# douban/gobeansdb

Hardware: AMD Instinct MI355X
Metric: GiB/s device-resident QuickLZ decompress (+compress), batched 4-64 KiB values (higher is better)
Workload: dtype u8; 1 GPU; c2: decompress 1048576 x 16384 B text-like blocks per GPU (ratio 0.502), device-resident; blocks_per_gpu=1048576, block_size=16384, unique_blocks=1048576, fused_crc=False, parallelism=shard1

## Files before the change

### gobeansdb_amd/csrc/qlzx_decode_batch.h

```cpp
#pragma once
#include "qlzx_device.h"

#ifndef QLZX_FAST_MAX_DSIZE
#define QLZX_FAST_MAX_DSIZE 65536
#endif

namespace qlzx {

struct BlkInfo {
    uint32_t ngroups;
    uint32_t nitems;
    uint32_t kind;
    uint32_t dsize;
};
struct GroupRec {
    uint32_t ip, m, a, b;
};

constexpr int32_t kPending = -1;
constexpr uint32_t kBlkSkip = 0, kBlkStored = 1, kBlkCompressed = 2;
constexpr uint32_t kParseWG = 64;
#ifndef QLZX_CHUNK_BLOCKS
#define QLZX_CHUNK_BLOCKS 262144
#endif
#ifndef QLZX_CHUNK_BLOCKS_MIXED
#define QLZX_CHUNK_BLOCKS_MIXED 131072
#endif
__host__ __device__ inline uint32_t chunk_blocks(uint32_t max_dsize) {
    return max_dsize <= 16384 ? (uint32_t)QLZX_CHUNK_BLOCKS : (uint32_t)QLZX_CHUNK_BLOCKS_MIXED;
}
constexpr uint32_t kRoundBytes = 32;
constexpr uint32_t kPieces = kRoundBytes / 16;
#ifndef QLZX_K1_SLOTS
#define QLZX_K1_SLOTS 4
#endif
constexpr uint32_t kRingSlots = QLZX_K1_SLOTS;
template <uint32_t S>
constexpr uint32_t kRingWaveS = S * kRoundBytes * 64;
__host__ __device__ inline uint32_t groups_max(uint32_t max_dsize) { return max_dsize / 31u + 2u; }

struct BatchLayout {
    uint32_t md, gmax;
    uint32_t chunk, nchunks;
    size_t o_rec, o_list, o_aux;
    size_t one;
    uint32_t regions;
};
inline BatchLayout batch_layout(uint32_t n, uint32_t max_dsize) {
    auto a256 = [](size_t x) { return (x + 255) & ~(size_t)255; };
    BatchLayout L;
    L.md = max_dsize > QLZX_FAST_MAX_DSIZE ? QLZX_FAST_MAX_DSIZE : max_dsize;
    L.gmax = groups_max(L.md);
    const uint32_t cb = chunk_blocks(max_dsize);
    L.chunk = n < cb ? (n ? n : 1) : cb;
    L.nchunks = n <= cb ? 1u : 1u + (n - 1) / cb;
    L.o_rec = a256((size_t)L.chunk * sizeof(BlkInfo));
    L.o_list = L.o_rec + a256((size_t)L.chunk * L.gmax * sizeof(GroupRec));
    L.o_aux = L.o_list + a256((size_t)n * sizeof(uint32_t));
    L.one = L.o_aux + 1024 + 256;
    L.regions = L.nchunks == 1 ? 1u : max_dsize > 16384 && L.nchunks >= 3 ? 3u : 2u;
    return L;
}

__device__ __forceinline__ int classify_block(const uint8_t *src, uint32_t len, uint32_t cap, uint32_t max_dsize,
                                              uint32_t &kind, uint32_t &csize, uint32_t &dsize, uint32_t &hdr) {
    kind = kBlkSkip;
    if (len < 3) return QLZX_E_HEADER;
    hdr = (src[0] & 2u) ? 9u : 3u;
    if (len < hdr) return QLZX_E_HEADER;
    const Header h = parse_header(src);
    csize = h.csize;
    dsize = h.dsize;
    if (h.csize != len) return QLZX_E_SIZE_COMPRESSED;
    if (h.level != 3) return QLZX_E_LEVEL;
    if (h.dsize > cap) return QLZX_E_DST_CAP;
    if (h.dsize > max_dsize) return QLZX_E_MAX_DSIZE;
    if (h.dsize > QLZX_FAST_MAX_DSIZE) return kPending;
    if (!h.compressed) {
        if (csize < hdr + dsize) return QLZX_E_CORRUPT;
        kind = kBlkStored;
    } else {
        kind = kBlkCompressed;
    }
    return QLZX_OK;
}

template <uint32_t S>
__device__ __forceinline__ uint32_t ring_off(uint32_t q, uint32_t lane) {
    return (((q >> 4) & (kPieces * S - 1)) << 10) | (lane << 4) | (q & 15u);
}
template <uint32_t S>
__device__ __forceinline__ uint32_t ring_rd32(const uint8_t *ring, uint32_t q, uint32_t lane) {
    const uint32_t qa = q & ~3u;
    const uint32_t lo = *(const uint32_t *)(ring + ring_off<S>(qa, lane));
    const uint32_t hi = *(const uint32_t *)(ring + ring_off<S>(qa + 4, lane));
    return __builtin_amdgcn_alignbyte(hi, lo, q & 3u);
}

struct ItemCursor {
    uint32_t g, k;
    __device__ __forceinline__ void next() {
        k += 2;
        const bool wrap = k >= 31;
        k = wrap ? k - 31 : k;
        g += wrap ? 3 : 2;
    }
};

__device__ __forceinline__ void decode_tok_bf(uint32_t t, uint32_t &off, uint32_t &len, uint32_t &tl) {
    const uint32_t ty = (t & 3u) + ((t & 127u) == 3u ? 1u : 0u);
    const uint32_t f4 = ty * 4, f6 = ty * 6;
    const uint32_t osh = __builtin_amdgcn_ubfe(0xF7622u, f4, 4);
    const uint32_t ow = __builtin_amdgcn_ubfe((6u) | (14u << 6) | (10u << 12) | (17u << 18) | (17u << 24), f6, 6);
    const uint32_t lsh = __builtin_amdgcn_ubfe(0x72200u, f4, 4);
    const uint32_t lw = __builtin_amdgcn_ubfe(0x85400u, f4, 4);
    const uint32_t la = __builtin_amdgcn_ubfe(0x32333u, f4, 4);
    tl = __builtin_amdgcn_ubfe(0x43221u, f4, 4);
    off = __builtin_amdgcn_ubfe(t, osh, ow);
    len = __builtin_amdgcn_ubfe(t, lsh, lw) + la;
}

__device__ __forceinline__ uint32_t wave_incl_scan(uint32_t v) {
    v += (uint32_t)__builtin_amdgcn_update_dpp(0, (int)v, 0x111, 0xf, 0xf, true);
    v += (uint32_t)__builtin_amdgcn_update_dpp(0, (int)v, 0x112, 0xf, 0xf, true);
    v += (uint32_t)__builtin_amdgcn_update_dpp(0, (int)v, 0x114, 0xf, 0xf, true);
    v += (uint32_t)__builtin_amdgcn_update_dpp(0, (int)v, 0x118, 0xf, 0xf, true);
    v += (uint32_t)__builtin_amdgcn_update_dpp(0, (int)v, 0x142, 0xa, 0xf, false);
    v += (uint32_t)__builtin_amdgcn_update_dpp(0, (int)v, 0x143, 0xc, 0xf, false);
    return v;
}

constexpr int kIcmpNe = 33, kIcmpUlt = 36;
__device__ __forceinline__ uint64_t cmp_lt(uint32_t a, uint32_t b) { return __builtin_amdgcn_uicmp(a, b, kIcmpUlt); }
__device__ __forceinline__ uint64_t cmp_ne(uint32_t a, uint32_t b) { return __builtin_amdgcn_uicmp(a, b, kIcmpNe); }
__device__ __forceinline__ bool in_mask(uint64_t m) { return __builtin_amdgcn_inverse_ballot_w64(m); }

__device__ __forceinline__ uint32_t ff1_or(uint64_t m, uint32_t dflt) {
    return m ? (uint32_t)__builtin_ctzll(m) : dflt;
}

__device__ __forceinline__ uint32_t wave_incl_max(uint32_t v) {
    v = max(v, (uint32_t)__builtin_amdgcn_update_dpp(0, (int)v, 0x111, 0xf, 0xf, false));
    v = max(v, (uint32_t)__builtin_amdgcn_update_dpp(0, (int)v, 0x112, 0xf, 0xf, false));
    v = max(v, (uint32_t)__builtin_amdgcn_update_dpp(0, (int)v, 0x114, 0xf, 0xf, false));
    v = max(v, (uint32_t)__builtin_amdgcn_update_dpp(0, (int)v, 0x118, 0xf, 0xf, false));
    v = max(v, (uint32_t)__builtin_amdgcn_update_dpp(0, (int)v, 0x142, 0xa, 0xf, false));
    v = max(v, (uint32_t)__builtin_amdgcn_update_dpp(0, (int)v, 0x143, 0xc, 0xf, false));
    return v;
}
__device__ __forceinline__ uint32_t wave_shr1(uint32_t v) {
    return (uint32_t)__builtin_amdgcn_update_dpp(0, (int)v, 0x138, 0xf, 0xf, true);
}

}
```

### gobeansdb_amd/csrc/qlzx_decode_batch.hip

```cpp
#include "qlzx_decode_batch.h"
#include "qlzx_decode_k2.h"
#include "qlzx_host.h"

namespace qlzx {

constexpr uint32_t kOrderClasses = 128, kOrderWG = 64, kOrderEPT = 16, kOrderPerWG = kOrderWG * kOrderEPT;
constexpr uint32_t kOrderAux = 2 * kOrderClasses;
__device__ __forceinline__ uint32_t order_class(uint32_t len) {
    const uint32_t c = len >> 9;
    return c < kOrderClasses - 1 ? c : kOrderClasses - 1;
}
__global__ void __launch_bounds__(kOrderWG) k_order_count(const uint32_t *src_len, uint32_t n, uint32_t *aux) {
    __shared__ uint32_t h[kOrderClasses];
    const uint32_t tid = threadIdx.x, i0 = blockIdx.x * kOrderPerWG + tid;
    for (uint32_t k = tid; k < kOrderClasses; k += kOrderWG) h[k] = 0;
    __syncthreads();
    uint32_t len[kOrderEPT];
#pragma unroll
    for (uint32_t e = 0; e < kOrderEPT; e++) {
        const uint32_t i = i0 + e * kOrderWG;
        len[e] = i < n ? src_len[i] : 0u;
    }
#pragma unroll
    for (uint32_t e = 0; e < kOrderEPT; e++)
        if (i0 + e * kOrderWG < n) atomicAdd(&h[order_class(len[e])], 1u);
    __syncthreads();
    for (uint32_t k = tid; k < kOrderClasses; k += kOrderWG)
        if (h[k]) atomicAdd(&aux[k], h[k]);
}
__global__ void __launch_bounds__(kOrderWG) k_order_scatter(const uint32_t *src_len, uint32_t n, uint32_t *aux,
                                                           uint32_t *list) {
    __shared__ uint32_t start[kOrderClasses], lc[kOrderClasses];
    const uint32_t tid = threadIdx.x, i0 = blockIdx.x * kOrderPerWG + tid;
    for (uint32_t k = tid; k < kOrderClasses; k += kOrderWG) start[k] = aux[k], lc[k] = 0;
    __syncthreads();
    if (tid == 0) {
        uint32_t acc = 0;
        for (uint32_t k = 0; k < kOrderClasses; k++) {
            const uint32_t v = start[k];
            start[k] = acc;
            acc += v;
        }
    }
    uint32_t c[kOrderEPT], r[kOrderEPT];
#pragma unroll
    for (uint32_t e = 0; e < kOrderEPT; e++) {
        const uint32_t i = i0 + e * kOrderWG;
        c[e] = i < n ? order_class(src_len[i]) : 0u;
    }
#pragma unroll
    for (uint32_t e = 0; e < kOrderEPT; e++)
        r[e] = (i0 + e * kOrderWG < n) ? atomicAdd(&lc[c[e]], 1u) : 0u;
    __syncthreads();
    for (uint32_t k = tid; k < kOrderClasses; k += kOrderWG)
        if (lc[k]) start[k] += atomicAdd(&aux[kOrderClasses + k], lc[k]);
    __syncthreads();
#pragma unroll
    for (uint32_t e = 0; e < kOrderEPT; e++)
        if (i0 + e * kOrderWG < n) list[start[c[e]] + r[e]] = i0 + e * kOrderWG;
}

#ifndef QLZX_K1_KMAX_UNI
#define QLZX_K1_KMAX_UNI 12
#endif
#ifndef QLZX_K1_KMAX_MIX
#define QLZX_K1_KMAX_MIX 10
#endif
int launch_k1_parse6(uint32_t grid, hipStream_t s, const qlzx_blocks &b, const uint32_t *dst_cap, uint32_t *dsize,
                     int32_t *status, uint32_t first, uint32_t cnt, BlkInfo *info, GroupRec *recs, uint32_t gmax,
                     const uint32_t *order, uint32_t max_dsize, uint32_t kmax);
int launch_k2_nocrc(uint32_t grid, hipStream_t s, const qlzx_blocks &b, uint32_t *dsize, int32_t *status,
                    uint32_t first, uint32_t cnt, const BlkInfo *info, const GroupRec *recs, uint32_t gmax,
                    const uint32_t *order);
inline std::atomic<int> g_batch_fault{0};
inline int batch_fault(int kernel) {
    int k = kernel;
    return g_batch_fault.load(std::memory_order_relaxed) == kernel && g_batch_fault.compare_exchange_strong(k, 0)
               ? (int)hipErrorLaunchFailure
               : 0;
}

struct Side {
    hipStream_t st = nullptr, st2 = nullptr;
    hipEvent_t k1[2] = {}, k2[2] = {}, order = nullptr, last = nullptr;
    ~Side() {
        if (!st || g_hip_down.load()) return;
        for (int j = 0; j < 2; j++) {
            if (k1[j]) (void)hipEventDestroy(k1[j]);
            if (k2[j]) (void)hipEventDestroy(k2[j]);
        }
        if (order) (void)hipEventDestroy(order);
        if (last) (void)hipEventDestroy(last);
        if (st2) (void)hipStreamDestroy(st2);
        (void)hipStreamDestroy(st);
    }
};
inline int batch_side(hipStream_t s, Side *&out) {
    thread_local Side sides[kMaxDevices];
    int dev = 0, cur = 0;
    if (s) {
        hipDevice_t hd;
        if (hipStreamGetDevice(s, &hd) != hipSuccess) return (int)hipErrorInvalidResourceHandle;
        dev = (int)hd;
    } else if (hipGetDevice(&dev) != hipSuccess) {
        return (int)hipErrorNoDevice;
    }
    if (dev < 0 || dev >= (int)kMaxDevices) return (int)hipErrorInvalidDevice;
    Side &sd = sides[dev];
    if (!sd.st) {
        note_hip_up();
        (void)hipGetDevice(&cur);
        if (cur != dev) (void)hipSetDevice(dev);
        hipError_t e = hipStreamCreateWithFlags(&sd.st, hipStreamNonBlocking);
        if (e == hipSuccess) e = hipStreamCreateWithFlags(&sd.st2, hipStreamNonBlocking);
        if (e == hipSuccess) e = hipEventCreateWithFlags(&sd.order, hipEventDisableTiming);
        if (e == hipSuccess) e = hipEventCreateWithFlags(&sd.last, hipEventDisableTiming);
        for (int j = 0; j < 2 && e == hipSuccess; j++) {
            e = hipEventCreateWithFlags(&sd.k1[j], hipEventDisableTiming);
            if (e == hipSuccess) e = hipEventCreateWithFlags(&sd.k2[j], hipEventDisableTiming);
        }
        if (cur != dev) (void)hipSetDevice(cur);
        if (e != hipSuccess) return (int)e;
    }
    out = &sd;
    return 0;
}

struct BatchCall {
    const qlzx_blocks &b;
    const uint32_t *dst_cap;
    uint32_t *dsize;
    int32_t *status;
    const uint32_t *crc_state, *crc_expect;
    uint32_t *crc_out;
    uint32_t max_dsize;
    uint8_t *ws;
    BatchLayout L;
    bool sort;

    BlkInfo *info(uint32_t region) const { return (BlkInfo *)(ws + region * L.one); }
    GroupRec *recs(uint32_t region) const { return (GroupRec *)(ws + region * L.one + L.o_rec); }
    uint32_t *order(uint32_t first) const { return sort ? (uint32_t *)(ws + L.o_list) + first : nullptr; }
};
inline int batch_k1(const BatchCall &c, hipStream_t st, uint32_t first, uint32_t cnt, uint32_t region) {
    if (const int ef = batch_fault(3)) return ef;
    return launch_k1_parse6((cnt + kParseWG - 1) / kParseWG, st, c.b, c.dst_cap, c.dsize, c.status, first, cnt,
                            c.info(region), c.recs(region), c.L.gmax, c.order(first), c.max_dsize,
                            c.max_dsize > 16384 ? (uint32_t)QLZX_K1_KMAX_MIX : (uint32_t)QLZX_K1_KMAX_UNI);
}
inline int batch_k2(const BatchCall &c, hipStream_t st, uint32_t first, uint32_t cnt, uint32_t region) {
    if (const int ef = batch_fault(4)) return ef;
    if (!(c.crc_state || c.crc_expect || c.crc_out))
        return launch_k2_nocrc(cnt, st, c.b, c.dsize, c.status, first, cnt, c.info(region), c.recs(region), c.L.gmax,
                               c.order(first));
    hipLaunchKernelGGL(k_dec_chunk4<true>, dim3(cnt), dim3(64), 0, st, c.b, c.dsize, c.status, first, cnt,
                       (const BlkInfo *)c.info(region), (const GroupRec *)c.recs(region), c.L.gmax,
                       (const uint32_t *)c.order(first), c.crc_state, c.crc_expect, c.crc_out);
    return 0;
}

inline int launch_decode_wave(const qlzx_blocks &b, const uint32_t *dst_cap, uint32_t *dsize,
                              int32_t *status, const uint32_t *crc_state, const uint32_t *crc_expect,
                              uint32_t *crc_out, uint32_t max_dsize, void *ws, size_t ws_bytes,
                              hipStream_t s) {
    const BatchLayout L = batch_layout(b.n, max_dsize);
    const BatchCall c{b, dst_cap, dsize, status, crc_state, crc_expect, crc_out, max_dsize, (uint8_t *)ws, L,
                      L.chunk > 64};
    const bool overlap = L.nchunks > 1 && ws_bytes >= 2 * L.one;
    Side *sd = nullptr;
    if (overlap)
        if (const int e = batch_side(s, sd)) return e;
    const bool split_k1 = overlap && max_dsize > 16384 && L.nchunks == 2;
    const bool early = overlap && L.regions == 3 && ws_bytes >= 3 * L.one;
    const uint32_t c_early = L.nchunks - (early ? 1 : 0);
    if (overlap) (void)hipEventRecord(sd->k2[1], s), (void)hipStreamWaitEvent(sd->st, sd->k2[1], 0);
    if (split_k1 || early) (void)hipStreamWaitEvent(sd->st2, sd->k2[1], 0);
    if (c.sort) {
        hipStream_t s1 = overlap ? sd->st : s;
        uint32_t *aux = (uint32_t *)(c.ws + L.o_aux);
        (void)hipMemsetAsync(aux, 0, kOrderAux * sizeof(uint32_t), s1);
        const dim3 g((b.n + kOrderPerWG - 1) / kOrderPerWG);
        hipLaunchKernelGGL(k_order_count, g, dim3(kOrderWG), 0, s1, b.src_len, b.n, aux);
        hipLaunchKernelGGL(k_order_scatter, g, dim3(kOrderWG), 0, s1, b.src_len, b.n, aux, c.order(0));
        if (split_k1 || early) (void)hipEventRecord(sd->order, sd->st), (void)hipStreamWaitEvent(sd->st2, sd->order, 0);
    }
    if (early) {
        const uint32_t fe = c_early * L.chunk;
        if (const int e1 = batch_k1(c, sd->st2, fe, b.n - fe, 2)) return e1;
        (void)hipEventRecord(sd->last, sd->st2);
    }
    uint32_t ci = 0;
    for (uint32_t first = 0, cnt = 0; first < b.n; first += cnt, ci++) {
        cnt = b.n - first < L.chunk ? b.n - first : L.chunk;
        const bool last_early = ci >= c_early;
        const uint32_t region = last_early ? 2 : overlap ? ci & 1 : 0;
        if (last_early) {
            (void)hipStreamWaitEvent(s, sd->last, 0);
        } else {
            hipStream_t s1 = overlap ? (split_k1 && (ci & 1) ? sd->st2 : sd->st) : s;
            if (overlap && ci >= 2) (void)hipStreamWaitEvent(s1, sd->k2[ci & 1], 0);
            if (const int e1 = batch_k1(c, s1, first, cnt, region)) return e1;
            if (overlap) (void)hipEventRecord(sd->k1[ci & 1], s1), (void)hipStreamWaitEvent(s, sd->k1[ci & 1], 0);
        }
        if (const int e2 = batch_k2(c, s, first, cnt, region)) return e2;
        if (overlap) (void)hipEventRecord(sd->k2[ci & 1], s);
        hipError_t e = hipGetLastError();
        if (e != hipSuccess) return (int)e;
    }
    return 0;
}

}
```

### gobeansdb_amd/csrc/qlzx_decode_k1.h

```cpp
#pragma once
#include "qlzx_decode_batch.h"

namespace qlzx {

__device__ __forceinline__ void k1_parse_wave(uint8_t *ring, uint32_t lane, uint32_t lin, const qlzx_blocks &b,
                                              const uint32_t *dst_cap, uint32_t *dsize_out, int32_t *status,
                                              uint32_t first, uint32_t count, BlkInfo *info, GroupRec *recs,
                                              uint32_t gmax, const uint32_t *order, uint32_t max_dsize,
                                              uint32_t kmax) {
    constexpr uint32_t S = kRingSlots;
    const bool inrange = lin < count;
    const uint32_t i = inrange ? (order ? order[lin] : first + lin) : first;

    int st = QLZX_OK;
    uint32_t kind = kBlkSkip, csize = 0, dsize = 0, hdr = 0, len = 0;
    const uint8_t *src = b.src + b.src_off[i];
    if (inrange) {
        len = b.src_len[i];
        st = classify_block(src, len, dst_cap ? dst_cap[i] : 0xffffffffu, max_dsize, kind, csize, dsize, hdr);
        if (st == QLZX_OK && kind == kBlkCompressed && dsize == 0) {
            st = (csize == hdr || csize == hdr + 9) ? QLZX_OK : QLZX_E_CORRUPT;
            kind = kBlkSkip;
        }
    }
    const uintptr_t a0 = (uintptr_t)src;
    const uint8_t *gbase = (const uint8_t *)(a0 & ~(uintptr_t)15);
    const uint32_t shift = (uint32_t)(a0 & 15);
    const uint32_t span = (st == QLZX_OK && kind == kBlkCompressed) ? csize : 0;
    const uint32_t last16 = span ? (span + shift - 1) >> 4 : 0;
    const uint32_t nrounds = span ? (span + shift - 1) / kRoundBytes + 1 : 0;
    const bool parsing = inrange && span > 0;

    uint32_t ip = hdr, g = 0, cwr = 1, cwg = 0, ra = 0, rb = 0, rec_ip = 0;
    GroupRec *myrec = recs + (size_t)(inrange ? lin : 0) * gmax;
    bool done_parse = !parsing;

    uint32_t rl = 0, ri = 0;
    constexpr uint32_t M = 2;
    static_assert(M == 2 || M == 3, "rounds per iteration");
    auto accept = [&]() __attribute__((always_inline)) -> uint32_t {
        const uint32_t cap = ((ip + shift) & ~3u) / kRoundBytes + S - 1;
        uint32_t n = 0;
#pragma unroll
        for (uint32_t k = 0; k < M; k++) n += (!done_parse && ri + k < nrounds && ri + k <= cap) ? 1u : 0u;
        return n;
    };
    typedef uint32_t u4v __attribute__((ext_vector_type(4)));
    typedef const __attribute__((address_space(1))) u4v g_u4;
    const uintptr_t gaddr = (uintptr_t)gbase;
#define K1_LD(n, k, j) (*(g_u4 *)(gaddr + (size_t)((n) > (k) ? min(ri * kPieces + 2 * (k) + (j), last16) : 0u) * 16))
#define K1_LOAD(n, v0, v1, v2, v3, v4, v5)                                                        \
    do {                                                                                          \
        v0 = K1_LD(n, 0, 0), v1 = K1_LD(n, 0, 1), v2 = K1_LD(n, 1, 0), v3 = K1_LD(n, 1, 1);        \
        if (M >= 3) v4 = K1_LD(n, 2, 0), v5 = K1_LD(n, 2, 1);                                     \
        ri += (n);                                                                                \
    } while (0)
#define K1_STORE(n, v0, v1, v2, v3, v4, v5)                                                       \
    do {                                                                                          \
                                 \
        asm volatile("" ::"v"(v0.x), "v"(v0.y), "v"(v0.z), "v"(v0.w), "v"(v1.x), "v"(v1.y),        \
                     "v"(v1.z), "v"(v1.w), "v"(v2.x), "v"(v2.y), "v"(v2.z), "v"(v2.w), "v"(v3.x),  \
                     "v"(v3.y), "v"(v3.z), "v"(v3.w));                                             \
        if (M >= 3) asm volatile("" ::"v"(v4.x), "v"(v4.y), "v"(v4.z), "v"(v4.w), "v"(v5.x),      \
                                 "v"(v5.y), "v"(v5.z), "v"(v5.w));                                 \
        uint8_t *sl0 = ring + (((rl & (S - 1)) * kPieces) << 10) + lane * 16;                     \
        uint8_t *sl1 = ring + ((((rl + 1) & (S - 1)) * kPieces) << 10) + lane * 16;               \
        uint8_t *sl2 = ring + ((((rl + 2) & (S - 1)) * kPieces) << 10) + lane * 16;               \
        if ((n) >= 1) *(u4v *)sl0 = v0, *(u4v *)(sl0 + 1024) = v1;                                \
        if ((n) >= 2) *(u4v *)sl1 = v2, *(u4v *)(sl1 + 1024) = v3;                                \
        if (M >= 3 && (n) >= 3) *(u4v *)sl2 = v4, *(u4v *)(sl2 + 1024) = v5;                      \
        rl += (n);                                                                                \
    } while (0)
    const uint32_t lane16 = lane << 4;
    auto rd32 = [&](uint32_t x) __attribute__((always_inline)) -> uint32_t {
        constexpr uint32_t PB = S * kPieces == 8 ? 3u : S * kPieces == 4 ? 2u : 4u;
        static_assert((1u << PB) == S * kPieces, "ring address below assumes 4, 8 or 16 pieces of 1 KiB");
        const uint32_t x4 = x + 4;
        const uint32_t a1 = (__builtin_amdgcn_ubfe(x, 4, PB) << 10) | ((x & 12u) | lane16);
        const uint32_t a2 = (__builtin_amdgcn_ubfe(x4, 4, PB) << 10) | ((x4 & 12u) | lane16);
        const uint32_t lo = *(const uint32_t *)(ring + a1);
        const uint32_t hi = *(const uint32_t *)(ring + a2);
        return __builtin_amdgcn_alignbyte(hi, lo, x);
    };
    auto tlc = [](uint32_t b) __attribute__((always_inline)) -> uint32_t {
        return __builtin_amdgcn_ubfe(0x94u, (b & 3u) * 2, 2) + ((b & 127u) == 3u ? 1u : 0u);
    };
    auto steps = [&]() __attribute__((always_inline)) -> uint32_t {
        const uint32_t lim = rl * kRoundBytes - shift;
        uint32_t k = 0;
        if (!done_parse) {
            for (;;) {
                const bool gb = cwr == 1;
                const uint32_t run = min((uint32_t)__builtin_ctz(cwr), csize - ip);
                const uint32_t q = ip + run;
                const uint32_t rest = cwr >> run;
                const bool hasm = (rest > 1u) & (q < csize);
                const uint32_t need = gb ? 4u : 1u;
                if (ip + need > csize) {
                    done_parse = true;
                    break;
                }
                if ((gb | hasm) & (q + need > lim)) break;
                const uint32_t w = rd32(q + shift);
                const uint32_t e = tlc(w);
                const uint32_t q2 = q + e + 1, rest2 = rest >> 1;
                const bool hasm2 = hasm & (e < 3u) & ((rest2 & 1u) != 0) & (rest2 > 1u) & (q2 < csize) & (q2 < lim);
                const uint32_t e2 = hasm2 ? tlc(__builtin_amdgcn_alignbyte(0u, w, e + 1)) : 0u;
                const bool bad = (gb & (((int32_t)w >= 0) | (g >= gmax))) | (hasm & (q2 > csize)) |
                                 (hasm2 & (q2 + e2 + 1 > csize));
                if (bad) {
                    if (gb) {
                        st = QLZX_E_CORRUPT;
                    } else {
                        const bool first = q2 <= csize;
                        const uint32_t idx = __builtin_clz(cwr) + run;
                        ra |= first ? (e & 1u) << idx : 0u;
                        rb |= first ? (e >> 1) << idx : 0u;
                        ip = first ? q2 : q;
                        cwr = rest >> (first ? 1u : 0u);
                    }
                    done_parse = true;
                    break;
                }
                if (gb) {
                    if (g > 0) {
                        typedef uint32_t u32x4 __attribute__((ext_vector_type(4)));
                        const u32x4 rec = {rec_ip, cwg, ra, rb};
                        asm volatile("global_store_dwordx4 %0, %1, off\n\ts_nop 1" ::"v"(myrec + (g - 1)), "v"(rec)
                                     : "memory");
                    }
                    rec_ip = ip;
                    cwg = w;
                    g++;
                    ip += 4;
                    cwr = w;
                    ra = 0;
                    rb = 0;
                } else {
                    const uint32_t idx = __builtin_clz(cwr) + run;
                    const uint32_t em = hasm ? e : 0u, e2m = hasm2 ? e2 : 0u;
                    ra |= ((em & 1u) | ((e2m & 1u) << 1)) << idx;
                    rb |= ((em >> 1) | (e2m & 2u)) << idx;
                    ip = q + em + e2m + (hasm ? 1u : 0u) + (hasm2 ? 1u : 0u);
                    cwr = rest >> ((hasm ? 1u : 0u) + (hasm2 ? 1u : 0u));
                }
                if (++k >= kmax) break;
            }
        }
        return k;
    };
#ifdef QLZX_PROFILE
    PROF_DECL
    auto k1prof = [&](uint32_t k) __attribute__((always_inline)) {
        uint32_t mx = k, sm = k;
        for (int o = 32; o >= 1; o >>= 1) {
            mx = max(mx, (uint32_t)__shfl_xor((int)mx, o));
            sm += (uint32_t)__shfl_xor((int)sm, o);
        }
        PROF_COUNT(0, 1);
        PROF_COUNT(1, mx);
        PROF_COUNT(2, sm);
    };
#define K1_STEPS() k1prof(steps())
#else
#define K1_STEPS() (void)steps()
#endif

    u4v pa0, pa1, pa2, pa3, pa4, pa5, pb0, pb1, pb2, pb3, pb4, pb5;
    uint32_t na = accept();
    K1_LOAD(na, pa0, pa1, pa2, pa3, pa4, pa5);
    uint32_t nb = 0;
    const uint32_t trip_cap = span + nrounds + 8;
    uint32_t trips = 0;
    auto guard = [&]() __attribute__((always_inline)) {
        trips++;
        if (!done_parse && trips > trip_cap) done_parse = true, st = QLZX_E_CORRUPT;
    };
    for (;;) {
        K1_STORE(na, pa0, pa1, pa2, pa3, pa4, pa5);
        nb = accept();
        K1_LOAD(nb, pb0, pb1, pb2, pb3, pb4, pb5);
        K1_STEPS();
        guard();
        if (__ballot(!done_parse) == 0) break;
        K1_STORE(nb, pb0, pb1, pb2, pb3, pb4, pb5);
        na = accept();
        K1_LOAD(na, pa0, pa1, pa2, pa3, pa4, pa5);
        K1_STEPS();
        guard();
        if (__ballot(!done_parse) == 0) break;
    }
#undef K1_LD
#undef K1_LOAD
#undef K1_STORE
#undef K1_STEPS
    if (parsing && st == QLZX_OK && g > 0) myrec[g - 1] = GroupRec{rec_ip, cwg, ra, rb};
    vm_sync();
#ifdef QLZX_PROFILE
    PROF_MARK(3);
    PROF_COUNT(4, 1);
    PROF_FLUSH(0);
#endif
    if (!inrange) return;
    if (st == QLZX_OK && kind == kBlkCompressed && (!done_parse || g == 0)) st = QLZX_E_CORRUPT;
    BlkInfo bi{0, 0, kind, dsize};
    if (st != QLZX_OK) {
        bi.kind = kBlkSkip;
        status[i] = st;
        if (dsize_out && st != kPending) dsize_out[i] = 0;
    } else if (kind == kBlkCompressed) {
        bi.ngroups = g;
        bi.nitems = (g - 1) * 31 + __builtin_clz(cwr);
    } else if (kind == kBlkSkip) {
        status[i] = QLZX_OK;
        if (dsize_out) dsize_out[i] = 0;
    }
    info[lin] = bi;
}

__global__ void __launch_bounds__(kParseWG) k_dec_parse6(qlzx_blocks b, const uint32_t *dst_cap, uint32_t *dsize_out,
                                                     int32_t *status, uint32_t first, uint32_t count, BlkInfo *info,
                                                     GroupRec *recs, uint32_t gmax, const uint32_t *order,
                                                     uint32_t max_dsize, uint32_t kmax) {
    constexpr uint32_t S = kRingSlots;
    __shared__ __attribute__((aligned(16))) uint8_t ring_all[(kParseWG / 64) * kRingWaveS<S>];
    const uint32_t lane = threadIdx.x & 63;
    uint8_t *ring = ring_all + (threadIdx.x >> 6) * kRingWaveS<S>;
    k1_parse_wave(ring, lane, blockIdx.x * kParseWG + threadIdx.x, b, dst_cap, dsize_out, status, first, count, info,
                  recs, gmax, order, max_dsize, kmax);
}

}
```

### gobeansdb_amd/csrc/qlzx_decode_k2.h

```cpp
#pragma once
#include "qlzx_crc.h"
#include "qlzx_decode_batch.h"

namespace qlzx {

constexpr uint32_t kV4W = 4096;
constexpr uint32_t kV4MR = 256;
constexpr uint32_t kV4Bpl = 4;
constexpr uint32_t kV4Chunk = 64 * kV4Bpl;
static_assert(kV4Chunk <= kV4MR, "a chunk's pointer-jumping array lives in its marker slots");

template <uint32_t W = kV4W>
struct K2v4Lds {
    uint8_t win[W];
    uint32_t mk[kV4MR];
};

template <uint32_t WIN>
__device__ __forceinline__ void dec_v4_block(K2v4Lds<WIN> &L, const uint8_t *src, uint8_t *dst, uint32_t csize,
                                             const BlkInfo bi, const GroupRec *rb, int32_t *status_i,
                                             uint32_t *dsize_i, uint32_t lane) {
    constexpr uint32_t W = WIN, MR = kV4MR, CH = kV4Chunk;
    const uint32_t dsize = bi.dsize;
    if (bi.kind == kBlkStored) {
        const uint32_t hdr = (src[0] & 2u) ? 9u : 3u;
        const uint8_t *s = src + hdr;
        uint32_t p0 = 0;
        if ((((uintptr_t)dst) & 15u) == 0) {
            p0 = dsize & ~15u;
            for (uint32_t p = lane * 16; p < p0; p += 1024) {
                const uint32_t *q = (const uint32_t *)(s + p);
                *(uint4 *)(dst + p) = make_uint4(q[0], q[1], q[2], q[3]);
            }
        }
        for (uint32_t p = p0 + lane; p < dsize; p += 64) dst[p] = s[p];
        if (lane == 0) { *status_i = QLZX_OK; if (dsize_i) *dsize_i = dsize; }
        return;
    }
    for (uint32_t q = lane * 4; q < MR; q += 256) *(uint4 *)(L.mk + q) = make_uint4(0, 0, 0, 0);

    const uint32_t nitems = bi.nitems;
    const uint32_t hdr = (src[0] & 2u) ? 9u : 3u;
    const uint32_t nb = (nitems + 63) / 64;
    const uint32_t tail_from = dsize > QLZX_TAIL ? dsize - 1 - QLZX_TAIL : 0;

    auto tok_pos = [&](const GroupRec &gr, const ItemCursor &c, uint32_t &p) -> uint32_t {
        const uint32_t low = (1u << c.k) - 1u;
        const uint32_t pos = gr.ip + 4 + c.k + __builtin_popcount(gr.a & low) + 2 * __builtin_popcount(gr.b & low);
        p = min(pos, csize - 4);
        return (pos & 0x7fffffffu) | (((gr.m >> c.k) & 1u) << 31);
    };
    const uint32_t glast = bi.ngroups - 1;
    ItemCursor ck{lane / 31, lane % 31};
    uint32_t posmA, tokA, posmB = 0, tokB = 0;
    GroupRec grA, grB;
    {
        const GroupRec g0 = rb[min(ck.g, glast)];
        uint32_t tp;
        posmA = tok_pos(g0, ck, tp);
        tokA = *(const uint32_t *)(src + tp);
        ck.next();
        grB = rb[min(ck.g, glast)];
        grA = grB;
    }
    PROF_DECL
    uint32_t D = 0, bt = 0, c = 0, cin = 0;
    bool tail = false, complete = false, err = false;
    uint64_t pendm = 0;
    uint32_t pd = 0, pkey = 0;
    uint32_t plit = 0;

    auto batch = [&](uint32_t posm, uint32_t tok, const GroupRec &gr_next, uint32_t &posm_n, uint32_t &tok_n,
                     GroupRec &gr_nn) __attribute__((always_inline)) {
        if (pendm) {
            if (in_mask(pendm)) {
                L.mk[pd & (MR - 1)] = pkey;
                if (plit < 0x100u) L.win[pd & (W - 1)] = (uint8_t)plit;
            }
            pendm = 0;
        }
        const uint64_t vm = cmp_lt(lane, nitems - bt * 64);
        const bool v = in_mask(vm);
        {
            uint32_t tp;
            posm_n = tok_pos(gr_next, ck, tp);
            tok_n = *(const uint32_t *)(src + tp);
            ck.next();
            gr_nn = rb[min(ck.g, glast)];
        }
        const uint64_t ismm = vm & cmp_ne(posm >> 31, 0u);
        const bool ism = in_mask(ismm);
        const uint32_t pos = posm & 0x7fffffffu;
        const uint32_t t = __builtin_amdgcn_alignbyte(0u, tok, __builtin_elementwise_sub_sat(pos, csize - 4));
        uint32_t off, mlen, tl;
        decode_tok_bf(t, off, mlen, tl);
        const uint32_t len = ism ? mlen : (v ? 1u : 0u);
        const uint32_t incl = wave_incl_scan(len);
        const uint32_t total = __builtin_amdgcn_readfirstlane(__builtin_amdgcn_readlane(incl, 63));
        const uint32_t d = D + incl - len;
        const uint64_t livem = vm & cmp_lt(d, dsize);
        const bool live = in_mask(livem);
        uint64_t badm;
        if (tail || D + total > tail_from) {
            tl = ism ? tl : 1u;
            const uint64_t tail_lanes = __ballot(live && !ism && d >= tail_from);
            const uint32_t tail_lane = tail ? 0u : ff1_or(tail_lanes, 64u);
            tail = tail || tail_lanes != 0;
            const bool mok = off >= 3 && off <= d && d + len + 4 <= dsize && lane < tail_lane;
            const bool last = live && d + len == dsize;
            const uint32_t ip_end = pos + tl;
            const bool eok = ip_end == csize || (ip_end < hdr + 9 && csize == hdr + 9);
            badm = __ballot(live && ((ism && !mok) || (last && !eok)));
            complete = __ballot(last) != 0;
        } else {
            badm = ismm & (cmp_lt(off, 3u) | cmp_lt(d, off));
        }
        if (badm) {
            err = true;
            return;
        }
        const uint32_t key = (d << 16) | (ism ? off : 0u);
        const uint64_t wrm = livem & cmp_lt(d, c + MR);
        if (in_mask(wrm)) {
            L.mk[d & (MR - 1)] = key;
            L.win[d & (W - 1)] = (uint8_t)t;
        }
        pendm = livem & ~wrm;
        pd = d;
        pkey = key;
        plit = ism ? 0x100u : (t & 0xffu);
        D = __builtin_amdgcn_readfirstlane(D + total);
        bt++;
        PROF_COUNT(5, 1);
    };

    auto chunks = [&]() __attribute__((always_inline)) -> bool {
        while (c < dsize && (complete || D >= c + CH)) {
            if (pendm) {
                const uint64_t wrm = pendm & cmp_lt(pd, c + MR);
                if (in_mask(wrm)) {
                    L.mk[pd & (MR - 1)] = pkey;
                    if (plit < 0x100u) L.win[pd & (W - 1)] = (uint8_t)plit;
                }
                pendm &= ~wrm;
            }
            constexpr uint32_t B = kV4Bpl;
            const uint32_t r0 = B * lane, p0 = c + r0;
            uint32_t *mkl = L.mk + ((c & (MR - 1)) + r0);
            uint32_t m[B];
#pragma unroll
            for (uint32_t h = 0; h < B; h += 4) {
                const uint4 q = *(const uint4 *)(mkl + h);
                m[h] = q.x, m[h + 1] = q.y, m[h + 2] = q.z, m[h + 3] = q.w;
            }
            uint32_t lmax = m[0];
#pragma unroll
            for (uint32_t j = 1; j < B; j++) lmax = max(lmax, m[j]);
            const uint32_t incl = wave_incl_max(lmax);
            uint32_t f = max(wave_shr1(incl), cin);
            cin = max(cin, (uint32_t)__builtin_amdgcn_readfirstlane(__builtin_amdgcn_readlane(incl, 63)));
            uint32_t rj[B];
            bool qa[B], anyq = false;
#pragma unroll
            for (uint32_t j = 0; j < B; j++) {
                f = max(f, m[j]);
                rj[j] = r0 + j - (f & 0xffffu);
                qa[j] = rj[j] < r0 + j;
                anyq = anyq || qa[j];
            }
            PROF_MARK(1);
            if (__ballot(anyq)) {
                uint32_t *spb = L.mk + (c & (MR - 1));
#pragma unroll
                for (uint32_t h = 0; h < B; h += 4) *(uint4 *)(mkl + h) = make_uint4(rj[h], rj[h + 1], rj[h + 2], rj[h + 3]);
                do {
                    uint32_t t[B];
#pragma unroll
                    for (uint32_t j = 0; j < B; j++) t[j] = spb[qa[j] ? rj[j] : r0 + j];
                    uint64_t anym = 0;
#pragma unroll
                    for (uint32_t j = 0; j < B; j++) {
                        qa[j] = t[j] < rj[j];
                        anym |= __ballot(qa[j]);
                        rj[j] = t[j];
                    }
                    anyq = anym != 0;
#pragma unroll
                    for (uint32_t h = 0; h < B; h += 4)
                        *(uint4 *)(mkl + h) = make_uint4(rj[h], rj[h + 1], rj[h + 2], rj[h + 3]);
                    PROF_COUNT(7, 1);
                } while (anyq);

            }
            PROF_MARK(2);
            const int32_t lo_rel = c + MR > W ? (int32_t)MR - (int32_t)W : -(int32_t)c;
            uint32_t vb[B], sv[B];
#pragma unroll
            for (uint32_t j = 0; j < B; j++) {
                sv[j] = rj[j] + c;
                vb[j] = L.win[sv[j] & (W - 1)];
            }
            int32_t mn = (int32_t)rj[0];
#pragma unroll
            for (uint32_t j = 1; j < B; j++) mn = min(mn, (int32_t)rj[j]);
            const bool far = mn < lo_rel;
            const uint32_t lo = c + lo_rel;
            PROF_COUNT(6, __ballot(far) ? 1 : 0);
            uint32_t w[B / 4];
            if (__ballot(far)) {
#pragma unroll
                for (uint32_t j = 0; j < B; j++)
                    if (sv[j] < lo) vb[j] = dst[sv[j]];
            }
#pragma unroll
            for (uint32_t h = 0; h < B / 4; h++)
                w[h] = vb[4 * h] | (vb[4 * h + 1] << 8) | (vb[4 * h + 2] << 16) | (vb[4 * h + 3] << 24);
            *(uint32_t *)(L.win + (p0 & (W - 1))) = w[0];
#pragma unroll
            for (uint32_t h = 0; h < B; h += 4) *(uint4 *)(mkl + h) = make_uint4(0, 0, 0, 0);
            PROF_MARK(3);
            if (c + CH <= dsize) {
                *(uint32_t *)(dst + p0) = w[0];
            } else {
                for (uint32_t j = 0; j < B && p0 + j < dsize; j++) dst[p0 + j] = (uint8_t)(w[j >> 2] >> (8 * (j & 3)));
            }
            c += CH;
            PROF_MARK(4);
        }
        return c >= dsize;
    };

    for (;;) {
        if (bt >= nb) { err = true; break; }
        batch(posmA, tokA, grB, posmB, tokB, grA);
        PROF_MARK(0);
        if (err || chunks()) break;
        if (bt >= nb) { err = true; break; }
        batch(posmB, tokB, grA, posmA, tokA, grB);
        PROF_MARK(0);
        if (err || chunks()) break;
    }
    vm_sync();
    PROF_FLUSH(1);
    if (lane == 0) {
        *status_i = err ? QLZX_E_CORRUPT : QLZX_OK;
        if (dsize_i) *dsize_i = err ? 0u : dsize;
    }
}

template <bool CRC, uint32_t WIN = kV4W>
__global__ void __launch_bounds__(64) k_dec_chunk4(qlzx_blocks b, uint32_t *dsize_out, int32_t *status,
                                                   uint32_t first, uint32_t count, const BlkInfo *info,
                                                   const GroupRec *recs, uint32_t gmax, const uint32_t *list,
                                                   const uint32_t *crc_state, const uint32_t *crc_expect,
                                                   uint32_t *crc_out) {
    __shared__ __attribute__((aligned(16))) K2v4Lds<WIN> L;
    const uint32_t bx = blockIdx.x;
    if (bx >= count) return;
    const uint32_t i = list ? list[bx] : first + bx;
    if constexpr (CRC) {
        static_assert(sizeof(K2v4Lds<WIN>) >= 4096, "the slicing-by-4 CRC tables fill 4 KiB of the window");
        const uint32_t lane = threadIdx.x;
        uint32_t *tab = (uint32_t *)&L;
        for (uint32_t e = lane * 4; e < 1024; e += 256) *(uint4 *)(tab + e) = *(const uint4 *)(g_crc_slice8 + e);
        __syncthreads();
        const uint32_t c = ~wave_crc_rep<4, 1>(tab, g_crc_mul, b.src + b.src_off[i], b.src_len[i],
                                                crc_state ? crc_state[i] : 0xffffffffu, lane);
        __syncthreads();
        if (lane == 0 && crc_out) crc_out[i] = c;
        if (crc_expect && c != crc_expect[i]) {
            if (lane == 0) {
                status[i] = QLZX_E_CRC;
                if (dsize_out) dsize_out[i] = 0;
            }
            return;
        }
    }
    const BlkInfo bi = info[bx];
    if (bi.kind == kBlkSkip) return;
    dec_v4_block(L, b.src + b.src_off[i], b.dst + b.dst_off[i], b.src_len[i], bi, recs + (size_t)bx * gmax,
                 status + i, dsize_out ? dsize_out + i : nullptr, threadIdx.x);
}

}
```

Baseline: 667.8 GiB/s.

## Pack block descriptor with index and length; scalar-load descriptors in decode kernel

Repacks BlkInfo so one 16-byte descriptor carries the block index, compressed length, packed dsize/ngroups/kind/header flag, and item count. The decode kernel reads it with a single scalar (constant address space) load and reads src/dst offsets the same way. This removes the list indirection, the src_len and header-byte reads, and the dependent global loads at kernel start. It also issues the first two group records before entering the block decoder. Error paths in the batch driver now join the side streams back to the main stream. The packing caps dsize at 17 bits and ngroups at 12, and the descriptor format changes between the parse and decode kernels.

Result: no change. 671.2 GiB/s, median of 6 (+0.5%).

```diff
diff --git a/gobeansdb_amd/csrc/qlzx_decode_batch.h b/gobeansdb_amd/csrc/qlzx_decode_batch.h
--- a/gobeansdb_amd/csrc/qlzx_decode_batch.h
+++ b/gobeansdb_amd/csrc/qlzx_decode_batch.h
@@ -7,18 +7,25 @@
 
 namespace qlzx {
 
+constexpr uint32_t kBlkSkip = 0, kBlkStored = 1, kBlkCompressed = 2;
 struct BlkInfo {
-    uint32_t ngroups;
-    uint32_t nitems;
-    uint32_t kind;
-    uint32_t dsize;
+    uint32_t i, len, w2, nitems;
+    __device__ __forceinline__ uint32_t dsize() const { return w2 & 0x1ffffu; }
+    __device__ __forceinline__ uint32_t ngroups() const { return (w2 >> 17) & 0xfffu; }
+    __device__ __forceinline__ uint32_t kind() const { return (w2 >> 29) & 3u; }
+    __device__ __forceinline__ uint32_t hdr() const { return (w2 >> 31) ? 9u : 3u; }
+    __device__ static __forceinline__ uint32_t pack(uint32_t dsize, uint32_t ngroups, uint32_t kind, uint32_t hdr) {
+        return dsize | (ngroups << 17) | (kind << 29) | (hdr == 9u ? 1u << 31 : 0u);
+    }
 };
+static_assert(sizeof(BlkInfo) == 16, "one dwordx4 per block; the workspace layout is part of the ABI");
+static_assert(QLZX_FAST_MAX_DSIZE < (1u << 17) && QLZX_FAST_MAX_DSIZE / 31u + 2u < (1u << 12),
+              "dsize takes 17 bits of a descriptor, ngroups 12");
 struct GroupRec {
     uint32_t ip, m, a, b;
 };
 
 constexpr int32_t kPending = -1;
-constexpr uint32_t kBlkSkip = 0, kBlkStored = 1, kBlkCompressed = 2;
 constexpr uint32_t kParseWG = 64;
 #ifndef QLZX_CHUNK_BLOCKS
 #define QLZX_CHUNK_BLOCKS 262144
diff --git a/gobeansdb_amd/csrc/qlzx_decode_batch.hip b/gobeansdb_amd/csrc/qlzx_decode_batch.hip
--- a/gobeansdb_amd/csrc/qlzx_decode_batch.hip
+++ b/gobeansdb_amd/csrc/qlzx_decode_batch.hip
@@ -173,6 +173,12 @@
     const bool split_k1 = overlap && max_dsize > 16384 && L.nchunks == 2;
     const bool early = overlap && L.regions == 3 && ws_bytes >= 3 * L.one;
     const uint32_t c_early = L.nchunks - (early ? 1 : 0);
+    bool on_st = false, on_st2 = false;
+    auto fail = [&](int e) {
+        if (on_st) (void)hipEventRecord(sd->order, sd->st), (void)hipStreamWaitEvent(s, sd->order, 0);
+        if (on_st2) (void)hipEventRecord(sd->last, sd->st2), (void)hipStreamWaitEvent(s, sd->last, 0);
+        return e;
+    };
     if (overlap) (void)hipEventRecord(sd->k2[1], s), (void)hipStreamWaitEvent(sd->st, sd->k2[1], 0);
     if (split_k1 || early) (void)hipStreamWaitEvent(sd->st2, sd->k2[1], 0);
     if (c.sort) {
@@ -182,11 +188,13 @@
         const dim3 g((b.n + kOrderPerWG - 1) / kOrderPerWG);
         hipLaunchKernelGGL(k_order_count, g, dim3(kOrderWG), 0, s1, b.src_len, b.n, aux);
         hipLaunchKernelGGL(k_order_scatter, g, dim3(kOrderWG), 0, s1, b.src_len, b.n, aux, c.order(0));
+        on_st = overlap;
         if (split_k1 || early) (void)hipEventRecord(sd->order, sd->st), (void)hipStreamWaitEvent(sd->st2, sd->order, 0);
     }
     if (early) {
         const uint32_t fe = c_early * L.chunk;
-        if (const int e1 = batch_k1(c, sd->st2, fe, b.n - fe, 2)) return e1;
+        if (const int e1 = batch_k1(c, sd->st2, fe, b.n - fe, 2)) return fail(e1);
+        on_st2 = true;
         (void)hipEventRecord(sd->last, sd->st2);
     }
     uint32_t ci = 0;
@@ -199,13 +207,14 @@
         } else {
             hipStream_t s1 = overlap ? (split_k1 && (ci & 1) ? sd->st2 : sd->st) : s;
             if (overlap && ci >= 2) (void)hipStreamWaitEvent(s1, sd->k2[ci & 1], 0);
-            if (const int e1 = batch_k1(c, s1, first, cnt, region)) return e1;
+            if (const int e1 = batch_k1(c, s1, first, cnt, region)) return fail(e1);
+            if (overlap) (s1 == sd->st ? on_st : on_st2) = true;
             if (overlap) (void)hipEventRecord(sd->k1[ci & 1], s1), (void)hipStreamWaitEvent(s, sd->k1[ci & 1], 0);
         }
-        if (const int e2 = batch_k2(c, s, first, cnt, region)) return e2;
+        if (const int e2 = batch_k2(c, s, first, cnt, region)) return fail(e2);
         if (overlap) (void)hipEventRecord(sd->k2[ci & 1], s);
         hipError_t e = hipGetLastError();
-        if (e != hipSuccess) return (int)e;
+        if (e != hipSuccess) return fail((int)e);
     }
     return 0;
 }
diff --git a/gobeansdb_amd/csrc/qlzx_decode_k1.h b/gobeansdb_amd/csrc/qlzx_decode_k1.h
--- a/gobeansdb_amd/csrc/qlzx_decode_k1.h
+++ b/gobeansdb_amd/csrc/qlzx_decode_k1.h
@@ -203,15 +203,17 @@
 #endif
     if (!inrange) return;
     if (st == QLZX_OK && kind == kBlkCompressed && (!done_parse || g == 0)) st = QLZX_E_CORRUPT;
-    BlkInfo bi{0, 0, kind, dsize};
+    BlkInfo bi{i, csize, 0, 0};
     if (st != QLZX_OK) {
-        bi.kind = kBlkSkip;
+        bi.len = b.src_len[i];
         status[i] = st;
         if (dsize_out && st != kPending) dsize_out[i] = 0;
     } else if (kind == kBlkCompressed) {
-        bi.ngroups = g;
+        bi.w2 = BlkInfo::pack(dsize, g, kBlkCompressed, hdr);
         bi.nitems = (g - 1) * 31 + __builtin_clz(cwr);
-    } else if (kind == kBlkSkip) {
+    } else if (kind == kBlkStored) {
+        bi.w2 = BlkInfo::pack(dsize, 0, kBlkStored, hdr);
+    } else {
         status[i] = QLZX_OK;
         if (dsize_out) dsize_out[i] = 0;
     }
diff --git a/gobeansdb_amd/csrc/qlzx_decode_k2.h b/gobeansdb_amd/csrc/qlzx_decode_k2.h
--- a/gobeansdb_amd/csrc/qlzx_decode_k2.h
+++ b/gobeansdb_amd/csrc/qlzx_decode_k2.h
@@ -16,14 +16,17 @@
     uint32_t mk[kV4MR];
 };
 
+struct BlkView {
+    uint32_t ngroups, nitems, kind, dsize;
+};
 template <uint32_t WIN>
 __device__ __forceinline__ void dec_v4_block(K2v4Lds<WIN> &L, const uint8_t *src, uint8_t *dst, uint32_t csize,
-                                             const BlkInfo bi, const GroupRec *rb, int32_t *status_i,
+                                             uint32_t hdr, const BlkView bi, const GroupRec &g0, const GroupRec &g1,
+                                             const GroupRec *rb, int32_t *status_i,
                                              uint32_t *dsize_i, uint32_t lane) {
     constexpr uint32_t W = WIN, MR = kV4MR, CH = kV4Chunk;
     const uint32_t dsize = bi.dsize;
     if (bi.kind == kBlkStored) {
-        const uint32_t hdr = (src[0] & 2u) ? 9u : 3u;
         const uint8_t *s = src + hdr;
         uint32_t p0 = 0;
         if ((((uintptr_t)dst) & 15u) == 0) {
@@ -40,7 +43,6 @@
     for (uint32_t q = lane * 4; q < MR; q += 256) *(uint4 *)(L.mk + q) = make_uint4(0, 0, 0, 0);
 
     const uint32_t nitems = bi.nitems;
-    const uint32_t hdr = (src[0] & 2u) ? 9u : 3u;
     const uint32_t nb = (nitems + 63) / 64;
     const uint32_t tail_from = dsize > QLZX_TAIL ? dsize - 1 - QLZX_TAIL : 0;
 
@@ -55,12 +57,11 @@
     uint32_t posmA, tokA, posmB = 0, tokB = 0;
     GroupRec grA, grB;
     {
-        const GroupRec g0 = rb[min(ck.g, glast)];
         uint32_t tp;
         posmA = tok_pos(g0, ck, tp);
         tokA = *(const uint32_t *)(src + tp);
         ck.next();
-        grB = rb[min(ck.g, glast)];
+        grB = g1;
         grA = grB;
     }
     PROF_DECL
@@ -248,6 +249,7 @@
     }
 }
 
+#define k2_pin(...) asm volatile("" ::__VA_ARGS__)
 template <bool CRC, uint32_t WIN = kV4W>
 __global__ void __launch_bounds__(64) k_dec_chunk4(qlzx_blocks b, uint32_t *dsize_out, int32_t *status,
                                                    uint32_t first, uint32_t count, const BlkInfo *info,
@@ -256,15 +258,23 @@
                                                    uint32_t *crc_out) {
     __shared__ __attribute__((aligned(16))) K2v4Lds<WIN> L;
     const uint32_t bx = blockIdx.x;
+    if constexpr (!CRC)
+        k2_pin("s"(b.src), "s"(b.src_off), "s"(b.dst), "s"(b.dst_off), "s"(dsize_out), "s"(status), "s"(count),
+           "s"(info), "s"(recs), "s"(gmax));
     if (bx >= count) return;
-    const uint32_t i = list ? list[bx] : first + bx;
+    const GroupRec *rb = recs + (size_t)bx * gmax;
+    typedef uint32_t k2_u32x4 __attribute__((ext_vector_type(4)));
+    const k2_u32x4 d = *(const __attribute__((address_space(4))) k2_u32x4 *)(uintptr_t)(info + bx);
+    const BlkInfo bi{d.x, d.y, d.z, d.w};
+    if constexpr (!CRC) k2_pin("s"(bi.i), "s"(bi.len), "s"(bi.w2), "s"(bi.nitems));
+    const uint32_t i = bi.i;
     if constexpr (CRC) {
         static_assert(sizeof(K2v4Lds<WIN>) >= 4096, "the slicing-by-4 CRC tables fill 4 KiB of the window");
         const uint32_t lane = threadIdx.x;
         uint32_t *tab = (uint32_t *)&L;
         for (uint32_t e = lane * 4; e < 1024; e += 256) *(uint4 *)(tab + e) = *(const uint4 *)(g_crc_slice8 + e);
         __syncthreads();
-        const uint32_t c = ~wave_crc_rep<4, 1>(tab, g_crc_mul, b.src + b.src_off[i], b.src_len[i],
+        const uint32_t c = ~wave_crc_rep<4, 1>(tab, g_crc_mul, b.src + b.src_off[i], bi.len,
                                                 crc_state ? crc_state[i] : 0xffffffffu, lane);
         __syncthreads();
         if (lane == 0 && crc_out) crc_out[i] = c;
@@ -276,10 +286,21 @@
             return;
         }
     }
-    const BlkInfo bi = info[bx];
-    if (bi.kind == kBlkSkip) return;
-    dec_v4_block(L, b.src + b.src_off[i], b.dst + b.dst_off[i], b.src_len[i], bi, recs + (size_t)bx * gmax,
-                 status + i, dsize_out ? dsize_out + i : nullptr, threadIdx.x);
+    if (bi.kind() == kBlkSkip) return;
+    GroupRec g0, g1;
+    {
+        const uint32_t glast = bi.ngroups() ? bi.ngroups() - 1 : 0;
+        ItemCursor ck{threadIdx.x / 31, threadIdx.x % 31};
+        g0 = rb[min(ck.g, glast)];
+        ck.next();
+        g1 = rb[min(ck.g, glast)];
+    }
+    typedef const __attribute__((address_space(4))) uint64_t c_u64;
+    const uint64_t so = *(c_u64 *)(uintptr_t)(b.src_off + i), dof = *(c_u64 *)(uintptr_t)(b.dst_off + i);
+    if constexpr (!CRC) k2_pin("s"(so), "s"(dof));
+    dec_v4_block(L, b.src + so, b.dst + dof, bi.len, bi.hdr(), BlkView{bi.ngroups(), bi.nitems, bi.kind(), bi.dsize()},
+                 g0, g1, rb, status + i, dsize_out ? dsize_out + i : nullptr, threadIdx.x);
 }
+#undef k2_pin
 
 }
```
